# POSTECH-CVLab/RoDyGS

Hardware: AMD Instinct MI355X
Metric: train-step fps at 1M dynamic Gaussians / 1080p (fwd+bwd+Adam, one camera per GPU per step) (higher is better)
Workload: dtype f32; 1 GPU; 1000000 dynamic Gaussians + deformation MLP, 1920x1080, SH3, 100-frame synthetic video (BASELINE configs[2]); points=1000000, width=1920, height=1080, scene=uniform, frames=100, deferred_overflow_check=True, frame_order=orbit positions, bit-reversed, one_device=False, graph_replay=False, densify_stats=True, deterministic_backward=True, render_normal=True, parallelism=single GPU (frame-dp1), losses=photometric, sh_adam_in_backward=True, binning=bucket

## Files before the change

rodygs_amd/csrc/rdg_api.hip:

```cpp
#include "rdg_common.h"
#include <dlfcn.h>
#include <math.h>
#include <stdarg.h>
#include <stdio.h>
#include <string.h>
#include <stdlib.h>
#include <mutex>

static thread_local char g_err[512] = "";

int rdg_set_error(const char* fmt, ...) {
    va_list ap;
    va_start(ap, fmt);
    vsnprintf(g_err, sizeof(g_err), fmt, ap);
    va_end(ap);
    return -1;
}
int rdg_check_hip(hipError_t e, const char* what) {
    if (e == hipSuccess) return 0;
    return rdg_set_error("%s: %s", what, hipGetErrorString(e));
}

#define RDG_MAX_PENDING 4096
struct RdgPending { hipEvent_t a, b; int stage; };
// ... 57 lines not shown
    if (stage < 0 || stage >= RDG_STAGE_COUNT || !g_open[stage]) return;
    hipEvent_t e;
    if (hipEventCreate(&e) != hipSuccess) { (void)hipEventDestroy(g_open[stage]); g_open[stage] = nullptr; return; }
    (void)hipEventRecord(e, s);
    std::lock_guard<std::mutex> lk(g_timing_mu);
    if (g_npending >= RDG_MAX_PENDING) rdg_timing_drain();
    g_pending[g_npending].a = g_open[stage];
    g_pending[g_npending].b = e;
    g_pending[g_npending].stage = stage;
    g_npending++;
    g_open[stage] = nullptr;
}

void rdg_set_pose_aux(hipStream_t s);
int rdg_pose_fork_event_ready();

static int rdg_make_dev(const RdgRasterSettings* s, RdgDev* d) {
    if (!s) return rdg_set_error("settings pointer is NULL");
    if (s->P < 0 || s->image_height <= 0 || s->image_width <= 0) return rdg_set_error("bad sizes");
    if (s->sh_degree < 0 || s->sh_degree > 3) return rdg_set_error("sh_degree must be 0..3");
    d->P = s->P; d->M = s->M; d->deg = s->sh_degree; d->H = s->image_height; d->W = s->image_width;
    d->gx = (d->W + RDG_TILE - 1) / RDG_TILE; d->gy = (d->H + RDG_TILE - 1) / RDG_TILE;
    d->tanx = s->tanfovx; d->tany = s->tanfovy;
    d->fx = (float)((double)d->W / (2.0 * (double)s->tanfovx));
    d->fy = (float)((double)d->H / (2.0 * (double)s->tanfovy));
    d->smod = s->scale_modifier;
    d->prefiltered = s->prefiltered; d->cov_grad = s->enable_cov_grad; d->sh_grad = s->enable_sh_grad;
    d->render_normal = s->render_normal;
    d->cull = s->cull ? 1 : 0;
    d->bin_mode = s->bin_mode; d->nren_stats = s->num_rendered_stats; d->list_hints = s->list_hints;
// ... 69 lines not shown
    size_t cap = (size_t)(capacity > 0 ? capacity : 1);
    return rdg_align_up(cap * 8, 256) + rdg_align_up(cap * 4, 256) + rdg_sort_layout(capacity).total;
}

int rdg_preprocess_forward(const RdgRasterSettings* s_host, const float* means3D, const float* shs,
                           const float* colors_precomp, const float* opacities, const float* scales,
                           const float* rotations, const float* cov3D_precomp, const float* viewmatrix,
                           const float* projmatrix, void* geom_ws, int32_t* radii, int32_t* num_rendered_dev,
                           void* stream) {
    RdgDev d;
    if (rdg_make_dev(s_host, &d)) return -1;
    if (rdg_check_inputs(s_host, shs, colors_precomp, scales, rotations, cov3D_precomp)) return -1;
    hipStream_t st = (hipStream_t)stream;
    rdg_stage_begin(RDG_STAGE_PREPROCESS, st);
    int rc = rdg_launch_preprocess_fwd(d, means3D, shs, colors_precomp, opacities, scales, rotations, cov3D_precomp,
                                       viewmatrix, projmatrix, geom_ws, radii, num_rendered_dev, st);
    rdg_stage_end(RDG_STAGE_PREPROCESS, st);
    return rc;
}

int rdg_geom_from_records(const RdgRasterSettings* s_host, void* geom_ws, int32_t* radii, int32_t* num_rendered_dev,
                          void* stream) {
    RdgDev d;
    if (rdg_make_dev(s_host, &d)) return -1;
    if (!geom_ws || !radii || !num_rendered_dev) return rdg_set_error("rdg_geom_from_records: NULL argument");
    return rdg_launch_geom_from_records(d, geom_ws, radii, num_rendered_dev, (hipStream_t)stream);
}

int rdg_composite_forward(const RdgRasterSettings* s_host, const float* bg, const void* geom_ws, const int32_t* radii,
                          void* binning_ws, int64_t capacity, void* image_ws, int32_t* num_rendered_dev,
                          float* out_color, float* out_depth, float* out_normal, float* out_alpha, void* stream) {
// ... 8 lines not shown
    rdg_stage_end(RDG_STAGE_RENDER_FWD, st);
    return rc;
}

int rdg_rasterize_forward(const RdgRasterSettings* s_host, const float* bg, const float* means3D, const float* shs,
                          const float* colors_precomp, const float* opacities, const float* scales,
                          const float* rotations, const float* cov3D_precomp, const float* viewmatrix,
                          const float* projmatrix, void* geom_ws, void* binning_ws, int64_t capacity, void* image_ws,
                          float* out_color, float* out_depth, float* out_normal, float* out_alpha, int32_t* radii,
                          int32_t* num_rendered_dev, void* stream) {
    RdgDev d;
    if (rdg_make_dev(s_host, &d)) return -1;
    if (rdg_check_inputs(s_host, shs, colors_precomp, scales, rotations, cov3D_precomp)) return -1;
    hipStream_t st = (hipStream_t)stream;
    const RdgImageLayout I = rdg_image_layout(d.H, d.W);
    rdg_stage_begin(RDG_STAGE_PREPROCESS, st);
    int rc = rdg_launch_preprocess_fwd(d, means3D, shs, colors_precomp, opacities, scales, rotations, cov3D_precomp,
                                       viewmatrix, projmatrix, geom_ws, radii, num_rendered_dev, st,
                                       (uint32_t*)((char*)image_ws + I.tile_cnt), rdg_cnt_entries(d.gx, d.gy));
    rdg_stage_end(RDG_STAGE_PREPROCESS, st);
    if (rc) return rc;
    d.tile_cnt_zeroed = 1;
    rc = rdg_launch_bin(d, geom_ws, radii, binning_ws, capacity, image_ws, num_rendered_dev, nullptr, nullptr, st);
    if (rc) return rc;
    rdg_stage_begin(RDG_STAGE_RENDER_FWD, st);
    rc = rdg_launch_render_fwd(d, bg, geom_ws, binning_ws, capacity, image_ws, num_rendered_dev, out_color, out_depth,
                               out_normal, out_alpha, st);
    rdg_stage_end(RDG_STAGE_RENDER_FWD, st);
    return rc;
}

int rdg_composite_backward(const RdgRasterSettings* s_host, const float* bg, const void* geom_ws,
                           const void* binning_ws, int64_t capacity, const void* image_ws,
                           const float* grad_out_color, const float* grad_out_depth, const float* grad_out_alpha,
                           const float* grad_out_normal, void* grad_ws, void* stream) {
    RdgDev d;
    if (rdg_make_dev(s_host, &d)) return -1;
    hipStream_t st = (hipStream_t)stream;
// ... 354 lines not shown
```

rodygs_amd/csrc/rdg_common.h:

```cpp
#pragma once
#include <hip/hip_runtime.h>
#include <stdint.h>
#include <stddef.h>
#include "../../include/rodygs_hip.h"

#define RDG_TILE 16
#define RDG_TILE_PIX 256
#define RDG_WAVE 64

#define RDG_NEAR_CULL 0.2f
#define RDG_FOV_CLAMP 1.3f
#define RDG_DILATION 0.3f
#define RDG_ALPHA_CAP 0.99f
#define RDG_ALPHA_MIN (1.0f / 255.0f)
#define RDG_T_STOP 0.0001f
#define RDG_LAMBDA_FLOOR 0.1f

struct __attribute__((aligned(64))) RdgRec {
    float4 q0, q1, q2, q3;
};

#define RDG_GROW 16

static inline size_t rdg_align_up(size_t x, size_t a) { return (x + a - 1) / a * a; }
// ... 190 lines not shown
__device__ __forceinline__ RdgShAdam rdg_sh_adam_resolve(RdgShAdam ad) {
    if (ad.dev) {
        const float inv = ad.dev->inv_bias_correction1;
        const bool tab = ad.dev->lr_from_table != 0;
        ad.step_head = (tab ? ad.dev->sh_lr_head : ad.lr_head) * inv;
        ad.step_tail = (tab ? ad.dev->sh_lr_tail : ad.lr_tail) * inv;
        ad.bc2_sqrt = ad.dev->sqrt_bias_correction2;
    }
    return ad;
}
#endif

int rdg_launch_preprocess_fwd(const RdgDev& d, const float* means3D, const float* shs, const float* colors,
                              const float* opac, const float* scales, const float* rots, const float* cov3D,
                              const float* view, const float* proj, void* geom_ws, int32_t* radii,
                              int32_t* num_rendered, hipStream_t s, uint32_t* zero_buf = nullptr, size_t zero_words = 0);
int rdg_launch_densify_stats(long long n, long long row0, const float* dmeans2D, const int32_t* radii, float* accum,
                             float* denom, float* maxr, hipStream_t s);
int rdg_launch_geom_from_records(const RdgDev& d, void* geom_ws, int32_t* radii, int32_t* num_rendered,
                                 hipStream_t s);
int rdg_launch_bin(const RdgDev& d, const void* geom_ws, const int32_t* radii, void* bin_ws, int64_t capacity,
                   void* image_ws, int32_t* num_rendered, uint64_t* keys_unsorted_copy,
                   uint32_t* vals_unsorted_copy, hipStream_t s, bool export_sorted_keys = false);
int rdg_launch_sort(uint64_t* keys_a, uint64_t* keys_b, uint32_t* vals_a, uint32_t* vals_b, int64_t capacity,
                    const int32_t* n_dev, int end_bit, void* sort_tmp, int* result_in_b, hipStream_t s);
template <typename KeyT>
int rdg_launch_radix_sort(KeyT* keys_a, KeyT* keys_b, uint32_t* vals_a, uint32_t* vals_b, int64_t capacity,
                        const int32_t* n_dev, int begin_bit, int end_bit, void* tmp, int* result_in_b, hipStream_t s);
int rdg_launch_render_fwd(const RdgDev& d, const float* bg, const void* geom_ws, void* bin_ws,
                          int64_t capacity, void* image_ws, const int32_t* num_rendered, float* out_color,
                          float* out_depth, float* out_normal, float* out_alpha, hipStream_t s);
// ... 265 lines not shown
```

rodygs_amd/csrc/rdg_preprocess_fwd.hip:

```cpp
#include "rdg_common.h"

#define SH_C0 0.28209479177387814f
#define SH_C1 0.4886025119029199f
__device__ static const float SH_C2[5] = {1.0925484305920792f, -1.0925484305920792f, 0.31539156525252005f,
                                          -1.0925484305920792f, 0.5462742152960396f};
__device__ static const float SH_C3[7] = {-0.5900435899266435f, 2.890611442640554f, -0.4570457994644658f,
                                          0.3731763325901154f,  -0.4570457994644658f, 1.445305721320277f,
                                          -0.5900435899266435f};

__device__ __forceinline__ void rdg_rect(float px, float py, int radius, int gx, int gy, int& x0, int& y0,
                                         int& x1, int& y1) {
    float r = (float)radius;
    x0 = min(gx, max(0, (int)((px - r) / (float)RDG_TILE)));
    y0 = min(gy, max(0, (int)((py - r) / (float)RDG_TILE)));
    x1 = min(gx, max(0, (int)((((px + r) + (float)RDG_TILE) - 1.0f) / (float)RDG_TILE)));
    y1 = min(gy, max(0, (int)((((py + r) + (float)RDG_TILE) - 1.0f) / (float)RDG_TILE)));
}

__device__ __forceinline__ float rdg_ln_exact_ops(float x) {
    const uint32_t u = __float_as_uint(x);
    int e = (int)(u >> 23) - 127;
    float m = __uint_as_float((u & 0x007fffffu) | 0x3f800000u);
    if (m > 1.41421354f) { m = m * 0.5f; e += 1; }
    const float s = (m - 1.0f) / (m + 1.0f);
// ... 18 lines not shown
    const float cxx = (c_eff * cyy) / a;
    const float hx = sqrtf(r2 * cxx), hy = sqrtf(r2 * cyy);
    const float lox = fmaxf(ceilf(q0.x - hx), 0.0f), hix = fminf(floorf(q0.x + hx), (float)(gx * RDG_TILE - 1));
    const float loy = fmaxf(ceilf(q0.y - hy), 0.0f), hiy = fminf(floorf(q0.y + hy), (float)(gy * RDG_TILE - 1));
    if (hix < lox || hiy < loy) { x1 = x0; y1 = y0; return; }
    x0 = max(x0, (int)lox >> 4); x1 = min(x1, ((int)hix >> 4) + 1);
    y0 = max(y0, (int)loy >> 4); y1 = min(y1, ((int)hiy >> 4) + 1);
    if (x1 < x0) x1 = x0;
    if (y1 < y0) y1 = y0;
}
__device__ __forceinline__ uint4 rdg_pack_rectd(int x0, int y0, int x1, int y1, float depth, uint32_t tiles) {
    if (tiles == 0u) return make_uint4(0u, 0u, 0u, 0u);
    return make_uint4((uint32_t)x0 | ((uint32_t)y0 << 16), (uint32_t)x1 | ((uint32_t)y1 << 16), __float_as_uint(depth), tiles);
}

template <bool MULTI>
__global__ void __launch_bounds__(RDG_PRE_BLOCK)
rdg_preprocess_fwd_kernel(RdgDev d, const float* __restrict__ view_b, const float* __restrict__ proj,
                          const float* __restrict__ means3D_b, const float* __restrict__ shs,
                          const float* __restrict__ colors, const float* __restrict__ opac,
                          const float* __restrict__ scales, const float* __restrict__ rots_b,
                          const float* __restrict__ cov3Dp, RdgRec* __restrict__ rec_b,
                          uint32_t* __restrict__ tiles_touched_b, uint8_t* __restrict__ clampedm_b,
                          uint32_t* __restrict__ block_sums_b, int32_t* __restrict__ radii_b, int nviews_arg,
                          int vstride_arg, int blk0_arg, uint4* __restrict__ rectd_b) {
    const int nviews = MULTI ? nviews_arg : 1, vstride = MULTI ? vstride_arg : 0;
    const int bid = (MULTI ? blk0_arg : 0) + (int)blockIdx.x;
    const int i = bid * RDG_PRE_BLOCK + threadIdx.x;
    __shared__ float sSH[RDG_PRE_BLOCK / 64][64 * 49];
    const int sh_row = d.M * 3, sh_stride = sh_row | 1;
    const long long wave_first = (long long)bid * RDG_PRE_BLOCK + (threadIdx.x >> 6) * 64;
    if (shs && wave_first < d.P) {
        rdg_rows_to_lds(shs, wave_first, d.P, sh_row, sh_stride, sSH[threadIdx.x >> 6], threadIdx.x & 63);
        rdg_wave_lds_sync();
    }
    __shared__ uint32_t wsum[RDG_PRE_BLOCK / RDG_WAVE];
    for (int vw = 0; vw < nviews; ++vw) {
    const size_t vo = (size_t)vw * vstride;
    const float* __restrict__ view = view_b + 16 * vw;
    const float* __restrict__ means3D = means3D_b + vo * 3;
    const float* __restrict__ rots = rots_b ? rots_b + vo * 4 : nullptr;
    RdgRec* __restrict__ rec = rec_b + vo;
    uint32_t* __restrict__ tiles_touched = tiles_touched_b + vo;
    uint8_t* __restrict__ clampedm = clampedm_b + vo;
    int32_t* __restrict__ radii = radii_b + vo;
    uint32_t* __restrict__ block_sums = block_sums_b + vo / RDG_PRE_BLOCK;
    uint4* __restrict__ rectd = rectd_b + vo;
    float V[16], Pm[16];
#pragma unroll
    for (int k = 0; k < 16; ++k) { V[k] = view[k]; Pm[k] = proj[k]; }
    uint32_t my_tiles = 0;
    if (i < d.P) {
        int radius_out = 0;
        uint8_t cl = 0;
        uint4 rd = make_uint4(0u, 0u, 0u, 0u);
        RdgRec R;
        R.q0 = make_float4(0.f, 0.f, 0.f, 0.f);
        R.q1 = R.q0; R.q2 = R.q0; R.q3 = R.q0;
        const float x = means3D[3 * i + 0], y = means3D[3 * i + 1], z = means3D[3 * i + 2];
        const float vx = ((V[0] * x + V[4] * y) + V[8] * z) + V[12];
        const float vy = ((V[1] * x + V[5] * y) + V[9] * z) + V[13];
        const float vz = ((V[2] * x + V[6] * y) + V[10] * z) + V[14];
        bool valid = vz > RDG_NEAR_CULL;
        if (valid) {
            const float hx = ((Pm[0] * vx + Pm[4] * vy) + Pm[8] * vz) + Pm[12];
            const float hy = ((Pm[1] * vx + Pm[5] * vy) + Pm[9] * vz) + Pm[13];
            const float hw = ((Pm[3] * vx + Pm[7] * vy) + Pm[11] * vz) + Pm[15];
            const float pw = 1.0f / (hw + 1e-7f);
            const float ndc_x = hx * pw, ndc_y = hy * pw;

            float S00, S01, S02, S11, S12, S22;
            float nx = 0.f, ny = 0.f, nz = 0.f;
            if (cov3Dp) {
                S00 = cov3Dp[6 * i + 0]; S01 = cov3Dp[6 * i + 1]; S02 = cov3Dp[6 * i + 2];
                S11 = cov3Dp[6 * i + 3]; S12 = cov3Dp[6 * i + 4]; S22 = cov3Dp[6 * i + 5];
            } else {
                const float s0 = d.smod * scales[3 * i + 0], s1 = d.smod * scales[3 * i + 1],
                            s2 = d.smod * scales[3 * i + 2];
                const float4 q = reinterpret_cast<const float4*>(rots)[i];
                const float r = q.x, qx = q.y, qy = q.z, qz = q.w;
                const float R00 = 1.0f - 2.0f * (qy * qy + qz * qz), R01 = 2.0f * (qx * qy - r * qz),
                            R02 = 2.0f * (qx * qz + r * qy);
                const float R10 = 2.0f * (qx * qy + r * qz), R11 = 1.0f - 2.0f * (qx * qx + qz * qz),
                            R12 = 2.0f * (qy * qz - r * qx);
                const float R20 = 2.0f * (qx * qz - r * qy), R21 = 2.0f * (qy * qz + r * qx),
                            R22 = 1.0f - 2.0f * (qx * qx + qy * qy);
                const float L00 = R00 * s0, L01 = R01 * s1, L02 = R02 * s2;
                const float L10 = R10 * s0, L11 = R11 * s1, L12 = R12 * s2;
                const float L20 = R20 * s0, L21 = R21 * s1, L22 = R22 * s2;
                S00 = (L00 * L00 + L01 * L01) + L02 * L02;
                S01 = (L00 * L10 + L01 * L11) + L02 * L12;
                S02 = (L00 * L20 + L01 * L21) + L02 * L22;
                S11 = (L10 * L10 + L11 * L11) + L12 * L12;
                S12 = (L10 * L20 + L11 * L21) + L12 * L22;
                S22 = (L20 * L20 + L21 * L21) + L22 * L22;
                if (d.render_normal) {
                    const float sc0 = scales[3 * i + 0], sc1 = scales[3 * i + 1], sc2 = scales[3 * i + 2];
                    int k = 0; float sm = sc0;
                    if (sc1 < sm) { sm = sc1; k = 1; }
                    if (sc2 < sm) { sm = sc2; k = 2; }
                    const float n0 = k == 0 ? R00 : (k == 1 ? R01 : R02);
                    const float n1 = k == 0 ? R10 : (k == 1 ? R11 : R12);
                    const float n2 = k == 0 ? R20 : (k == 1 ? R21 : R22);
                    float nvx = (V[0] * n0 + V[4] * n1) + V[8] * n2;
                    float nvy = (V[1] * n0 + V[5] * n1) + V[9] * n2;
                    float nvz = (V[2] * n0 + V[6] * n1) + V[10] * n2;
                    const float dotv = (nvx * vx + nvy * vy) + nvz * vz;
                    const float sg = dotv > 0.f ? -1.0f : 1.0f;
                    nx = nvx * sg; ny = nvy * sg; nz = nvz * sg;
                }
            }
            const float limx = RDG_FOV_CLAMP * d.tanx, limy = RDG_FOV_CLAMP * d.tany;
// ... 12 lines not shown
            const float u12 = (T10 * S02 + T11 * S12) + T12 * S22;
            const float ca = ((u00 * T00 + u01 * T01) + u02 * T02) + RDG_DILATION;
            const float cb = (u00 * T10 + u01 * T11) + u02 * T12;
            const float cc = ((u10 * T10 + u11 * T11) + u12 * T12) + RDG_DILATION;
            const float det = ca * cc - cb * cb;
            valid = det != 0.0f;
            if (valid) {
                const float det_inv = 1.0f / det;
                const float mid = 0.5f * (ca + cc);
                const float disc = sqrtf(fmaxf(RDG_LAMBDA_FLOOR, mid * mid - det));
                const float lam = fmaxf(mid + disc, mid - disc);
                const int radius = (int)ceilf(3.0f * sqrtf(lam));
                const float px = ((ndc_x + 1.0f) * (float)d.W - 1.0f) * 0.5f;
                const float py = ((ndc_y + 1.0f) * (float)d.H - 1.0f) * 0.5f;
                const float4 rq0 = make_float4(px, py, cc * det_inv, -cb * det_inv);
                const float4 rq1 = make_float4(ca * det_inv, opac[i], vz, __int_as_float(radius));
                const float inv_cyy = 1.0f / cc;
                int x0, y0, x1, y1;
                rdg_rect(px, py, radius, d.gx, d.gy, x0, y0, x1, y1);
                const int area = (x1 - x0) * (y1 - y0);
                if (area > 0) {
                    if (d.cull) rdg_splat_rect(rq0, rq1, inv_cyy, d.gx, d.gy, 1, x0, y0, x1, y1);
                    my_tiles = (uint32_t)((x1 - x0) * (y1 - y0));
                    rd = rdg_pack_rectd(x0, y0, x1, y1, vz, my_tiles);
                    radius_out = radius;
                    float cr, cg, cbl;
                    if (colors) {
                        cr = colors[3 * i + 0]; cg = colors[3 * i + 1]; cbl = colors[3 * i + 2];
                    } else {
                        const float camx = -((V[0] * V[12] + V[1] * V[13]) + V[2] * V[14]);
                        const float camy = -((V[4] * V[12] + V[5] * V[13]) + V[6] * V[14]);
                        const float camz = -((V[8] * V[12] + V[9] * V[13]) + V[10] * V[14]);
                        float dx = x - camx, dy = y - camy, dz = z - camz;
                        const float ln = sqrtf((dx * dx + dy * dy) + dz * dz);
                        dx = dx / ln; dy = dy / ln; dz = dz / ln;
                        const float* sh = sSH[threadIdx.x >> 6] + (threadIdx.x & 63) * sh_stride;
                        float res[3];
#pragma unroll
                        for (int c = 0; c < 3; ++c) res[c] = SH_C0 * sh[c];
                        if (d.deg > 0) {
#pragma unroll
                            for (int c = 0; c < 3; ++c)
                                res[c] = res[c] - SH_C1 * dy * sh[3 + c] + SH_C1 * dz * sh[6 + c] -
                                         SH_C1 * dx * sh[9 + c];
                            if (d.deg > 1) {
                                const float xx = dx * dx, yy = dy * dy, zz = dz * dz;
                                const float xy = dx * dy, yz = dy * dz, xz = dx * dz;
#pragma unroll
                                for (int c = 0; c < 3; ++c)
                                    res[c] = res[c] + SH_C2[0] * xy * sh[12 + c] + SH_C2[1] * yz * sh[15 + c] +
                                             SH_C2[2] * (2.0f * zz - xx - yy) * sh[18 + c] +
                                             SH_C2[3] * xz * sh[21 + c] + SH_C2[4] * (xx - yy) * sh[24 + c];
                                if (d.deg > 2) {
#pragma unroll
                                    for (int c = 0; c < 3; ++c)
                                        res[c] = res[c] + SH_C3[0] * dy * (3.0f * xx - yy) * sh[27 + c] +
                                                 SH_C3[1] * xy * dz * sh[30 + c] +
                                                 SH_C3[2] * dy * (4.0f * zz - xx - yy) * sh[33 + c] +
                                                 SH_C3[3] * dz * (2.0f * zz - 3.0f * xx - 3.0f * yy) * sh[36 + c] +
                                                 SH_C3[4] * dx * (4.0f * zz - xx - yy) * sh[39 + c] +
                                                 SH_C3[5] * dz * (xx - yy) * sh[42 + c] +
                                                 SH_C3[6] * dx * (xx - 3.0f * yy) * sh[45 + c];
                                }
                            }
                        }
                        res[0] += 0.5f; res[1] += 0.5f; res[2] += 0.5f;
                        if (res[0] < 0.f) cl |= 1;
                        if (res[1] < 0.f) cl |= 2;
                        if (res[2] < 0.f) cl |= 4;
                        cr = fmaxf(res[0], 0.f); cg = fmaxf(res[1], 0.f); cbl = fmaxf(res[2], 0.f);
                    }
                    R.q0 = rq0;
                    R.q1 = rq1;
                    R.q2 = make_float4(cr, cg, cbl, inv_cyy);
                    R.q3 = make_float4(nx, ny, nz, 0.f);
                }
            }
        }
        rec[i] = R;
        tiles_touched[i] = my_tiles;
        rectd[i] = rd;
        clampedm[i] = cl;
        radii[i] = radius_out;
    }
    uint32_t inc = rdg_wave_scan_incl(my_tiles);
    const uint32_t lane = threadIdx.x & 63, w = threadIdx.x >> 6;
    if (lane == 63) wsum[w] = inc;
    __syncthreads();
    if (threadIdx.x == 0) block_sums[bid] = wsum[0] + wsum[1] + wsum[2] + wsum[3];
    if (nviews > 1) __syncthreads();
    }
}

__global__ void __launch_bounds__(1024) rdg_scan_block_sums_kernel(uint32_t* __restrict__ block_sums, int nblk,
                                                                   int32_t* __restrict__ num_rendered,
                                                                   uint32_t* __restrict__ zero_buf, int zero_words,
                                                                   int32_t* __restrict__ nren_max) {
    for (int i = threadIdx.x; i < zero_words; i += 1024) zero_buf[i] = 0u;
    __shared__ uint32_t wtot[16];
    __shared__ unsigned long long wtot64[16];
    const uint32_t lane = threadIdx.x & 63, w = threadIdx.x >> 6;
    const int per = (nblk + 1023) / 1024;
    const int t0 = min(nblk, (int)threadIdx.x * per), t1 = min(nblk, t0 + per);
    uint32_t mine = 0;
    unsigned long long mine64 = 0ull;
    for (int c0 = t0; c0 < t1; c0 += 8) {
// ... 68 lines not shown
    char* g = (char*)geom_ws;
    const int nblk = (d.P + RDG_PRE_BLOCK - 1) / RDG_PRE_BLOCK;
    uint32_t* block_sums = (uint32_t*)(g + L.block_sums);
    if (d.P > 0)
        hipLaunchKernelGGL(rdg_geom_from_records_kernel, dim3(nblk), dim3(RDG_PRE_BLOCK), 0, s, d.P, d.gx, d.gy, d.cull,
                           (const RdgRec*)(g + L.rec), (uint32_t*)(g + L.tiles_touched), block_sums, radii,
                           (uint4*)(g + L.rectd));
    hipLaunchKernelGGL(rdg_scan_block_sums_kernel, dim3(1), dim3(1024), 0, s, block_sums, d.P > 0 ? nblk : 0,
                       num_rendered, (uint32_t*)nullptr, 0, d.nren_max);
    return rdg_check_hip(hipGetLastError(), "geom_from_records launch");
}

int rdg_launch_preprocess_fwd(const RdgDev& d, const float* means3D, const float* shs, const float* colors,
                              const float* opac, const float* scales, const float* rots, const float* cov3D,
                              const float* view, const float* proj, void* geom_ws, int32_t* radii,
                              int32_t* num_rendered, hipStream_t s, uint32_t* zero_buf, size_t zero_words) {
    const RdgGeomLayout L = rdg_geom_layout(d.P);
    char* g = (char*)geom_ws;
    const int nblk = (d.P + RDG_PRE_BLOCK - 1) / RDG_PRE_BLOCK;
    uint32_t* block_sums = (uint32_t*)(g + L.block_sums);
    if (d.P > 0) {
        hipLaunchKernelGGL(rdg_preprocess_fwd_kernel<false>, dim3(nblk), dim3(RDG_PRE_BLOCK), 0, s, d, view, proj, means3D,
                           shs, colors, opac, scales, rots, cov3D, (RdgRec*)(g + L.rec),
                           (uint32_t*)(g + L.tiles_touched), (uint8_t*)(g + L.clamped), block_sums, radii, 1, 0, 0,
                           (uint4*)(g + L.rectd));
    }
    hipLaunchKernelGGL(rdg_scan_block_sums_kernel, dim3(1), dim3(1024), 0, s, block_sums, d.P > 0 ? nblk : 0,
                       num_rendered, zero_buf, (int)zero_words, d.nren_max);
    return rdg_check_hip(hipGetLastError(), "preprocess_fwd launch");
}

int rdg_launch_preprocess_fwd_views(const RdgDev& d_in, int32_t nviews, int32_t stride, int32_t row0,
                                    const float* means3D, const float* shs, const float* opac, const float* scales,
                                    const float* rots, const float* views, const float* proj, void* geom_ws,
                                    int32_t* radii, hipStream_t s) {
    const RdgGeomLayout L = rdg_geom_layout(nviews * stride);
// ... 13 lines not shown
```

rodygs_amd/rasterizer.py:

```python
from __future__ import annotations

import ctypes as C
import os
import threading
from typing import NamedTuple, Optional

import torch
import torch.nn as nn

from . import _lib

RENDER_NORMAL = True
PREZERO_GRAD_ROWS = os.environ.get("RDG_PREZERO_GRAD_ROWS", "1") != "0"
NREN_HOST_MIRROR = os.environ.get("RDG_NREN_MIRROR", "1") != "0"
BIN_RADIX_ABOVE = 32768
BIN_BUCKET_BELOW = 16384
BIN_RADIX_MEAN_LIST_ABOVE = 1000
BIN_BUCKET_MEAN_LIST_BELOW = 800
SPLIT_ABOVE = 4096
SPLIT_BELOW = 3072
_FORCE_RADIX = os.environ.get("RDG_BIN_MODE", "") == "radix"
_FORCE_BUCKET = os.environ.get("RDG_BIN_MODE", "") == "bucket"

DETERMINISTIC = os.environ.get("RDG_DETERMINISTIC", "0") == "1"
# ... 23 lines not shown
        self.capacity_hint = {}
        self.d_high = {}
        self.bin_hint = {}
        self.split_hint = {}
        self.pending = []
        self.pinned_free = []
        self.last_nren = None
        self.last_image = None
        self.graph_capture = False
        self.nren_max = None
        self.nren_max_key = None
        self.det_ws = None
        self.aux_stream = None
        self.pose_grad = None
        self.pose_fork_eager = None
        self.keep_alive = []
        self.lock = threading.RLock()

    def mode(self, name: str) -> bool:
        v = getattr(self, name)
        if v is not None:
            return bool(v)
        return bool({"deterministic": DETERMINISTIC, "force_radix": _FORCE_RADIX, "force_bucket": _FORCE_BUCKET,
                     "deferred_overflow_check": DEFERRED_OVERFLOW_CHECK, "render_normal": RENDER_NORMAL,
                     "cull": CULL}[name])

    def note_instances(self, key, n: int) -> None:
        self.d_high[key] = max(int(n), int(self.d_high.get(key, 0) * HINT_DECAY))

    def pinned_slot(self) -> torch.Tensor:
# ... 230 lines not shown
                cs.list_hints = 1 if det_mode else int(state.split_hint.get(key, 0))
                cap = max(int(state.capacity_hint.get(key, 0) * 1.25) + 4096, 4 * P + 4096)
                if capture and key not in state.capacity_hint:
                    raise RuntimeError("graph capture needs a warm-up forward of this (P, H, W) on the same RasterState first")
                deferred = state.mode("deferred_overflow_check") and key in state.capacity_hint and not capture
                if deferred:
                    state.poll_overflow(block=False)
                host = None
                if deferred:
                    host = state.pinned_slot()
                    host[0], host[1] = -1, -1
                    if NREN_HOST_MIRROR:
                        cs.num_rendered_host = host.data_ptr()
                if state.nren_max is not None and state.nren_max_key in (None, key):
                    cs.num_rendered_max = state.nren_max.data_ptr()
            while True:
                binning = torch.empty(L.rdg_binning_bytes(cap, n_tiles), **u8)
                rc = L.rdg_rasterize_forward(C.byref(cs), _lib.ptr(bg), _lib.ptr(m3), _lib.ptr(shs), _lib.ptr(col),
                                             _lib.ptr(op), _lib.ptr(sc), _lib.ptr(ro), _lib.ptr(cov), _lib.ptr(vm),
                                             _lib.ptr(pm), _lib.ptr(geom), _lib.ptr(binning), cap, _lib.ptr(image),
                                             _lib.ptr(color), _lib.ptr(depth), _lib.ptr(normal), _lib.ptr(alpha),
                                             _lib.ptr(radii), _lib.ptr(nren), stream)
                _lib.check(rc, "rdg_rasterize_forward")
                state.last_nren = (nren, key, cap)
                if capture:
                    n = -1
                    break
                if deferred:
                    if not NREN_HOST_MIRROR:
                        host.copy_(nren, non_blocking=True)
# ... 210 lines not shown
```

rodygs_amd/trainstep.py:

```python
from __future__ import annotations

import math
import os
from typing import Optional

import torch
import torch.nn.functional as F

from . import _lib
from .deform import (MLPBasisNetwork, dynamic_gaussians, dynamic_getter_supported, gaussian_deformation,
                     gaussian_deformation_packed)
from .dp import BucketedAllReduce, FlatParams, allreduce_sum_, frame_for
from .losses import fused_photometric_loss
from .model_ops import activate_gaussians, pose_view_matrix
from .rasterizer import GaussianRasterizationSettings, GaussianRasterizer, RasterState


def quaternion_to_matrix(q: torch.Tensor) -> torch.Tensor:
    r, i, j, k = q[0], q[1], q[2], q[3]
    two_s = 2.0 / (q * q).sum()
    return torch.stack([
        1 - two_s * (j * j + k * k), two_s * (i * j - k * r), two_s * (i * k + j * r),
        two_s * (i * j + k * r), 1 - two_s * (i * i + k * k), two_s * (j * k - i * r),
        two_s * (i * k - j * r), two_s * (j * k + i * r), 1 - two_s * (i * i + j * j)]).reshape(3, 3)
# ... 109 lines not shown
                h = ctypes.c_void_p()
                prio = int(os.environ.get("RDG_SIDE_STREAM_PRIORITY", str(least.value)))
                if hip.hipStreamCreateWithPriority(ctypes.byref(h), 1, prio) == 0 and h.value:
                    st = torch.cuda.ExternalStream(h.value, device=idx)
    except OSError:
        st = None
    if st is None:
        st = torch.cuda.Stream(device=idx)
    _LOW_PRIORITY_STREAMS[idx] = st
    return st


_FUSE_SH_ADAM = os.environ.get("RDG_FUSE_SH_ADAM", "1") != "0"
_EARLY_ROWS_ADAM = os.environ.get("RDG_EARLY_ROWS_ADAM", "1") != "0"
_EAGER_POSE_FORK = os.environ.get("RDG_EAGER_POSE_FORK", "1") != "0"
_PLAIN_FULL_FAST = os.environ.get("RDG_PLAIN_FULL_FAST", "1") != "0"

_MLP_SINK_ORDER = ("timenet.0.weight", "timenet.0.bias", "timenet.2.weight", "timenet.2.bias", "timenet.4.weight",
                   "timenet.4.bias", "head_w1", "head_b1", "head_w2", "head_b2")


def bind_module_to_flat(net: torch.nn.Module, lr: float, device, extra_spec=None) -> FlatParams:
    spec = {name: (tuple(p.shape), lr) for name, p in net.named_parameters()}
    spec.update(extra_spec or {})
    sp = FlatParams(spec, device)
    with torch.no_grad():
        for name, p in list(net.named_parameters()):
            sp[name].copy_(p)
            mod_name, _, leaf = name.rpartition(".")
            mod = net.get_submodule(mod_name) if mod_name else net
# ... 355 lines not shown
        main = torch.cuda.current_stream(self.device)
        if self._side_stream is None:
            self._side_stream = _low_priority_stream(self.device)
        side = self._side_stream
        side.wait_stream(main)
        with torch.cuda.stream(side):
            fused_adam_(self.fp, names=[k for k in self.fp.names if k != "features"])
        self._rows_stepped = True

    def train_step(self, step: int, rank: int = 0, world: int = 1, perm=None) -> torch.Tensor:
        perm = perm if perm is not None else list(self.gt.keys())
        frame = frame_for(step, rank, world, perm)
        after = None
        self._rows_adam_hook, self._rows_stepped = None, False
        self.raster_state.pose_fork_eager = None
        if self.full_losses and step % self.rigidity[1] != 0 and _PLAIN_FULL_FAST:
            fuse = world == 1 and _FUSE_SH_ADAM
            loss, after = self._full_loss_plain(frame, fuse)
        elif self.full_losses:
            loss = self._full_loss(step, frame)
        else:
            self.fuse_sh_adam = fuse = world == 1 and _FUSE_SH_ADAM
            eager = self._graph_inputs is None and not self.raster_state.graph_capture
            if fuse and _EARLY_ROWS_ADAM and eager:
                self._rows_adam_hook = self._step_rows_early
            if fuse and _EAGER_POSE_FORK and eager and self.pose_sinks is not None:
                if self._pose_fork is None:
                    self._pose_fork = (torch.cuda.Stream(device=self.device),
                                       torch.empty(4, 4, dtype=torch.float32, device=self.device))
                self.raster_state.pose_fork_eager = self._pose_fork
# ... 330 lines not shown
```

Before: 710.9 frames/s.

## Split SH colour evaluation from preprocess and overlap it with binning on aux stream

Splits the forward preprocess into a geometry-only kernel (no SH loads into LDS) and a separate colour kernel that evaluates SH for visible Gaussians. When an aux stream is available in eager mode, the colour kernel runs on that stream concurrently with binning, joined before render. The goal is to take the SH-to-RGB cost and its LDS footprint off the critical path. In exchange it adds an extra kernel launch, a second read of means, and event fork/join overhead, plus contention between streams.

```diff
diff --git a/rodygs_amd/csrc/rdg_api.hip b/rodygs_amd/csrc/rdg_api.hip
--- a/rodygs_amd/csrc/rdg_api.hip
+++ b/rodygs_amd/csrc/rdg_api.hip
@@ -95,6 +95,23 @@
 
 void rdg_set_pose_aux(hipStream_t s);
 int rdg_pose_fork_event_ready();
+
+static int rdg_fwd_split_colour() {
+    const char* e = getenv("RDG_FWD_SPLIT_COLOUR");
+    return e && e[0] == '0' ? 0 : (e && e[0] == '2' ? 2 : 1);
+}
+static thread_local hipEvent_t g_colour_fork_ev = nullptr, g_colour_join_ev = nullptr;
+static int rdg_colour_events_ready() {
+    if (!g_colour_fork_ev && hipEventCreateWithFlags(&g_colour_fork_ev, hipEventDisableTiming) != hipSuccess) {
+        g_colour_fork_ev = nullptr;
+        return rdg_set_error("colour fork: hipEventCreate failed");
+    }
+    if (!g_colour_join_ev && hipEventCreateWithFlags(&g_colour_join_ev, hipEventDisableTiming) != hipSuccess) {
+        g_colour_join_ev = nullptr;
+        return rdg_set_error("colour join: hipEventCreate failed");
+    }
+    return 0;
+}
 
 static int rdg_make_dev(const RdgRasterSettings* s, RdgDev* d) {
     if (!s) return rdg_set_error("settings pointer is NULL");
@@ -194,7 +211,8 @@
     hipStream_t st = (hipStream_t)stream;
     rdg_stage_begin(RDG_STAGE_PREPROCESS, st);
     int rc = rdg_launch_preprocess_fwd(d, means3D, shs, colors_precomp, opacities, scales, rotations, cov3D_precomp,
-                                       viewmatrix, projmatrix, geom_ws, radii, num_rendered_dev, st);
+                                       viewmatrix, projmatrix, geom_ws, radii, num_rendered_dev, st, nullptr, 0,
+                                       rdg_fwd_split_colour() == 2);
     rdg_stage_end(RDG_STAGE_PREPROCESS, st);
     return rc;
 }
@@ -233,14 +251,27 @@
     if (rdg_check_inputs(s_host, shs, colors_precomp, scales, rotations, cov3D_precomp)) return -1;
     hipStream_t st = (hipStream_t)stream;
     const RdgImageLayout I = rdg_image_layout(d.H, d.W);
+    const int split_mode = rdg_fwd_split_colour();
+    hipStream_t aux = nullptr;
+    if (split_mode && shs && !colors_precomp && d.P > 0 && s_host->aux_stream && (hipStream_t)s_host->aux_stream != st) {
+        hipStreamCaptureStatus cap_st = hipStreamCaptureStatusNone;
+        if (hipStreamIsCapturing(st, &cap_st) != hipSuccess) { (void)hipGetLastError(); cap_st = hipStreamCaptureStatusActive; }
+        if (cap_st == hipStreamCaptureStatusNone) {
+            if (rdg_colour_events_ready()) return -1;
+            aux = (hipStream_t)s_host->aux_stream;
+        }
+    }
+    const bool split = split_mode == 2 || aux != nullptr;
     rdg_stage_begin(RDG_STAGE_PREPROCESS, st);
     int rc = rdg_launch_preprocess_fwd(d, means3D, shs, colors_precomp, opacities, scales, rotations, cov3D_precomp,
                                        viewmatrix, projmatrix, geom_ws, radii, num_rendered_dev, st,
-                                       (uint32_t*)((char*)image_ws + I.tile_cnt), rdg_cnt_entries(d.gx, d.gy));
+                                       (uint32_t*)((char*)image_ws + I.tile_cnt), rdg_cnt_entries(d.gx, d.gy), split, aux,
+                                       g_colour_fork_ev, g_colour_join_ev);
     rdg_stage_end(RDG_STAGE_PREPROCESS, st);
-    if (rc) return rc;
+    if (rc) { if (aux) (void)hipStreamWaitEvent(st, g_colour_join_ev, 0); return rc; }
     d.tile_cnt_zeroed = 1;
     rc = rdg_launch_bin(d, geom_ws, radii, binning_ws, capacity, image_ws, num_rendered_dev, nullptr, nullptr, st);
+    if (aux && hipStreamWaitEvent(st, g_colour_join_ev, 0) != hipSuccess && !rc) rc = rdg_check_hip(hipGetLastError(), "colour join wait");
     if (rc) return rc;
     rdg_stage_begin(RDG_STAGE_RENDER_FWD, st);
     rc = rdg_launch_render_fwd(d, bg, geom_ws, binning_ws, capacity, image_ws, num_rendered_dev, out_color, out_depth,
diff --git a/rodygs_amd/csrc/rdg_common.h b/rodygs_amd/csrc/rdg_common.h
--- a/rodygs_amd/csrc/rdg_common.h
+++ b/rodygs_amd/csrc/rdg_common.h
@@ -228,7 +228,9 @@
 int rdg_launch_preprocess_fwd(const RdgDev& d, const float* means3D, const float* shs, const float* colors,
                               const float* opac, const float* scales, const float* rots, const float* cov3D,
                               const float* view, const float* proj, void* geom_ws, int32_t* radii,
-                              int32_t* num_rendered, hipStream_t s, uint32_t* zero_buf = nullptr, size_t zero_words = 0);
+                              int32_t* num_rendered, hipStream_t s, uint32_t* zero_buf = nullptr, size_t zero_words = 0,
+                              bool split_colour = false, hipStream_t colour_stream = nullptr, hipEvent_t fork_ev = nullptr,
+                              hipEvent_t join_ev = nullptr);
 int rdg_launch_densify_stats(long long n, long long row0, const float* dmeans2D, const int32_t* radii, float* accum,
                              float* denom, float* maxr, hipStream_t s);
 int rdg_launch_geom_from_records(const RdgDev& d, void* geom_ws, int32_t* radii, int32_t* num_rendered,
diff --git a/rodygs_amd/csrc/rdg_preprocess_fwd.hip b/rodygs_amd/csrc/rdg_preprocess_fwd.hip
--- a/rodygs_amd/csrc/rdg_preprocess_fwd.hip
+++ b/rodygs_amd/csrc/rdg_preprocess_fwd.hip
@@ -56,7 +56,53 @@
     return make_uint4((uint32_t)x0 | ((uint32_t)y0 << 16), (uint32_t)x1 | ((uint32_t)y1 << 16), __float_as_uint(depth), tiles);
 }
 
-template <bool MULTI>
+__device__ __forceinline__ uint8_t rdg_sh_to_rgb(int deg, const float (&V)[16], float x, float y, float z,
+                                                 const float* sh, float& cr, float& cg, float& cbl) {
+    const float camx = -((V[0] * V[12] + V[1] * V[13]) + V[2] * V[14]);
+    const float camy = -((V[4] * V[12] + V[5] * V[13]) + V[6] * V[14]);
+    const float camz = -((V[8] * V[12] + V[9] * V[13]) + V[10] * V[14]);
+    float dx = x - camx, dy = y - camy, dz = z - camz;
+    const float ln = sqrtf((dx * dx + dy * dy) + dz * dz);
+    dx = dx / ln; dy = dy / ln; dz = dz / ln;
+    float res[3];
+#pragma unroll
+    for (int c = 0; c < 3; ++c) res[c] = SH_C0 * sh[c];
+    if (deg > 0) {
+#pragma unroll
+        for (int c = 0; c < 3; ++c)
+            res[c] = res[c] - SH_C1 * dy * sh[3 + c] + SH_C1 * dz * sh[6 + c] -
+                     SH_C1 * dx * sh[9 + c];
+        if (deg > 1) {
+            const float xx = dx * dx, yy = dy * dy, zz = dz * dz;
+            const float xy = dx * dy, yz = dy * dz, xz = dx * dz;
+#pragma unroll
+            for (int c = 0; c < 3; ++c)
+                res[c] = res[c] + SH_C2[0] * xy * sh[12 + c] + SH_C2[1] * yz * sh[15 + c] +
+                         SH_C2[2] * (2.0f * zz - xx - yy) * sh[18 + c] +
+                         SH_C2[3] * xz * sh[21 + c] + SH_C2[4] * (xx - yy) * sh[24 + c];
+            if (deg > 2) {
+#pragma unroll
+                for (int c = 0; c < 3; ++c)
+                    res[c] = res[c] + SH_C3[0] * dy * (3.0f * xx - yy) * sh[27 + c] +
+                             SH_C3[1] * xy * dz * sh[30 + c] +
+                             SH_C3[2] * dy * (4.0f * zz - xx - yy) * sh[33 + c] +
+                             SH_C3[3] * dz * (2.0f * zz - 3.0f * xx - 3.0f * yy) * sh[36 + c] +
+                             SH_C3[4] * dx * (4.0f * zz - xx - yy) * sh[39 + c] +
+                             SH_C3[5] * dz * (xx - yy) * sh[42 + c] +
+                             SH_C3[6] * dx * (xx - 3.0f * yy) * sh[45 + c];
+            }
+        }
+    }
+    res[0] += 0.5f; res[1] += 0.5f; res[2] += 0.5f;
+    uint8_t cl = 0;
+    if (res[0] < 0.f) cl |= 1;
+    if (res[1] < 0.f) cl |= 2;
+    if (res[2] < 0.f) cl |= 4;
+    cr = fmaxf(res[0], 0.f); cg = fmaxf(res[1], 0.f); cbl = fmaxf(res[2], 0.f);
+    return cl;
+}
+
+template <bool MULTI, bool GEOM = false, bool COV = false>
 __global__ void __launch_bounds__(RDG_PRE_BLOCK)
 rdg_preprocess_fwd_kernel(RdgDev d, const float* __restrict__ view_b, const float* __restrict__ proj,
                           const float* __restrict__ means3D_b, const float* __restrict__ shs,
@@ -69,12 +115,15 @@
     const int nviews = MULTI ? nviews_arg : 1, vstride = MULTI ? vstride_arg : 0;
     const int bid = (MULTI ? blk0_arg : 0) + (int)blockIdx.x;
     const int i = bid * RDG_PRE_BLOCK + threadIdx.x;
-    __shared__ float sSH[RDG_PRE_BLOCK / 64][64 * 49];
+    static_assert(!(MULTI && GEOM), "the geometry kernel is single-camera");
+    __shared__ float sSH[GEOM ? 1 : RDG_PRE_BLOCK / 64][GEOM ? 1 : 64 * 49];
     const int sh_row = d.M * 3, sh_stride = sh_row | 1;
     const long long wave_first = (long long)bid * RDG_PRE_BLOCK + (threadIdx.x >> 6) * 64;
-    if (shs && wave_first < d.P) {
-        rdg_rows_to_lds(shs, wave_first, d.P, sh_row, sh_stride, sSH[threadIdx.x >> 6], threadIdx.x & 63);
-        rdg_wave_lds_sync();
+    if constexpr (!GEOM) {
+        if (shs && wave_first < d.P) {
+            rdg_rows_to_lds(shs, wave_first, d.P, sh_row, sh_stride, sSH[threadIdx.x >> 6], threadIdx.x & 63);
+            rdg_wave_lds_sync();
+        }
     }
     __shared__ uint32_t wsum[RDG_PRE_BLOCK / RDG_WAVE];
     for (int vw = 0; vw < nviews; ++vw) {
@@ -100,6 +149,25 @@
         R.q0 = make_float4(0.f, 0.f, 0.f, 0.f);
         R.q1 = R.q0; R.q2 = R.q0; R.q3 = R.q0;
         const float x = means3D[3 * i + 0], y = means3D[3 * i + 1], z = means3D[3 * i + 2];
+        float in_sc[3] = {0.f, 0.f, 0.f}, in_cov[6] = {0.f, 0.f, 0.f, 0.f, 0.f, 0.f}, in_op = 0.f;
+        float4 in_q = make_float4(0.f, 0.f, 0.f, 0.f);
+        const bool has_cov = GEOM ? COV : cov3Dp != nullptr;
+        if constexpr (GEOM) {
+            in_op = opac[i];
+            if constexpr (COV) {
+#pragma unroll
+                for (int k = 0; k < 6; ++k) in_cov[k] = cov3Dp[6 * i + k];
+            } else {
+                in_sc[0] = scales[3 * i + 0]; in_sc[1] = scales[3 * i + 1]; in_sc[2] = scales[3 * i + 2];
+                in_q = reinterpret_cast<const float4*>(rots)[i];
+            }
+            if constexpr (COV)
+                asm volatile("" ::"v"(in_op), "v"(in_cov[0]), "v"(in_cov[1]), "v"(in_cov[2]), "v"(in_cov[3]), "v"(in_cov[4]),
+                             "v"(in_cov[5]));
+            else
+                asm volatile("" ::"v"(in_op), "v"(in_sc[0]), "v"(in_sc[1]), "v"(in_sc[2]), "v"(in_q.x), "v"(in_q.y), "v"(in_q.z),
+                             "v"(in_q.w));
+        }
         const float vx = ((V[0] * x + V[4] * y) + V[8] * z) + V[12];
         const float vy = ((V[1] * x + V[5] * y) + V[9] * z) + V[13];
         const float vz = ((V[2] * x + V[6] * y) + V[10] * z) + V[14];
@@ -113,13 +181,20 @@
 
             float S00, S01, S02, S11, S12, S22;
             float nx = 0.f, ny = 0.f, nz = 0.f;
-            if (cov3Dp) {
-                S00 = cov3Dp[6 * i + 0]; S01 = cov3Dp[6 * i + 1]; S02 = cov3Dp[6 * i + 2];
-                S11 = cov3Dp[6 * i + 3]; S12 = cov3Dp[6 * i + 4]; S22 = cov3Dp[6 * i + 5];
+            if (has_cov) {
+                if constexpr (!GEOM) {
+#pragma unroll
+                    for (int k = 0; k < 6; ++k) in_cov[k] = cov3Dp[6 * i + k];
+                }
+                S00 = in_cov[0]; S01 = in_cov[1]; S02 = in_cov[2];
+                S11 = in_cov[3]; S12 = in_cov[4]; S22 = in_cov[5];
             } else {
-                const float s0 = d.smod * scales[3 * i + 0], s1 = d.smod * scales[3 * i + 1],
-                            s2 = d.smod * scales[3 * i + 2];
-                const float4 q = reinterpret_cast<const float4*>(rots)[i];
+                if constexpr (!GEOM) {
+                    in_sc[0] = scales[3 * i + 0]; in_sc[1] = scales[3 * i + 1]; in_sc[2] = scales[3 * i + 2];
+                    in_q = reinterpret_cast<const float4*>(rots)[i];
+                }
+                const float s0 = d.smod * in_sc[0], s1 = d.smod * in_sc[1], s2 = d.smod * in_sc[2];
+                const float4 q = in_q;
                 const float r = q.x, qx = q.y, qy = q.z, qz = q.w;
                 const float R00 = 1.0f - 2.0f * (qy * qy + qz * qz), R01 = 2.0f * (qx * qy - r * qz),
                             R02 = 2.0f * (qx * qz + r * qy);
@@ -137,7 +212,7 @@
                 S12 = (L10 * L20 + L11 * L21) + L12 * L22;
                 S22 = (L20 * L20 + L21 * L21) + L22 * L22;
                 if (d.render_normal) {
-                    const float sc0 = scales[3 * i + 0], sc1 = scales[3 * i + 1], sc2 = scales[3 * i + 2];
+                    const float sc0 = in_sc[0], sc1 = in_sc[1], sc2 = in_sc[2];
                     int k = 0; float sm = sc0;
                     if (sc1 < sm) { sm = sc1; k = 1; }
                     if (sc2 < sm) { sm = sc2; k = 2; }
@@ -180,7 +255,8 @@
                 const float px = ((ndc_x + 1.0f) * (float)d.W - 1.0f) * 0.5f;
                 const float py = ((ndc_y + 1.0f) * (float)d.H - 1.0f) * 0.5f;
                 const float4 rq0 = make_float4(px, py, cc * det_inv, -cb * det_inv);
-                const float4 rq1 = make_float4(ca * det_inv, opac[i], vz, __int_as_float(radius));
+                if constexpr (!GEOM) in_op = opac[i];
+                const float4 rq1 = make_float4(ca * det_inv, in_op, vz, __int_as_float(radius));
                 const float inv_cyy = 1.0f / cc;
                 int x0, y0, x1, y1;
                 rdg_rect(px, py, radius, d.gx, d.gy, x0, y0, x1, y1);
@@ -193,48 +269,11 @@
                     float cr, cg, cbl;
                     if (colors) {
                         cr = colors[3 * i + 0]; cg = colors[3 * i + 1]; cbl = colors[3 * i + 2];
+                    } else if constexpr (GEOM) {
+                        cr = cg = cbl = 0.f;
                     } else {
-                        const float camx = -((V[0] * V[12] + V[1] * V[13]) + V[2] * V[14]);
-                        const float camy = -((V[4] * V[12] + V[5] * V[13]) + V[6] * V[14]);
-                        const float camz = -((V[8] * V[12] + V[9] * V[13]) + V[10] * V[14]);
-                        float dx = x - camx, dy = y - camy, dz = z - camz;
-                        const float ln = sqrtf((dx * dx + dy * dy) + dz * dz);
-                        dx = dx / ln; dy = dy / ln; dz = dz / ln;
                         const float* sh = sSH[threadIdx.x >> 6] + (threadIdx.x & 63) * sh_stride;
-                        float res[3];
-#pragma unroll
-                        for (int c = 0; c < 3; ++c) res[c] = SH_C0 * sh[c];
-                        if (d.deg > 0) {
-#pragma unroll
-                            for (int c = 0; c < 3; ++c)
-                                res[c] = res[c] - SH_C1 * dy * sh[3 + c] + SH_C1 * dz * sh[6 + c] -
-                                         SH_C1 * dx * sh[9 + c];
-                            if (d.deg > 1) {
-                                const float xx = dx * dx, yy = dy * dy, zz = dz * dz;
-                                const float xy = dx * dy, yz = dy * dz, xz = dx * dz;
-#pragma unroll
-                                for (int c = 0; c < 3; ++c)
-                                    res[c] = res[c] + SH_C2[0] * xy * sh[12 + c] + SH_C2[1] * yz * sh[15 + c] +
-                                             SH_C2[2] * (2.0f * zz - xx - yy) * sh[18 + c] +
-                                             SH_C2[3] * xz * sh[21 + c] + SH_C2[4] * (xx - yy) * sh[24 + c];
-                                if (d.deg > 2) {
-#pragma unroll
-                                    for (int c = 0; c < 3; ++c)
-                                        res[c] = res[c] + SH_C3[0] * dy * (3.0f * xx - yy) * sh[27 + c] +
-                                                 SH_C3[1] * xy * dz * sh[30 + c] +
-                                                 SH_C3[2] * dy * (4.0f * zz - xx - yy) * sh[33 + c] +
-                                                 SH_C3[3] * dz * (2.0f * zz - 3.0f * xx - 3.0f * yy) * sh[36 + c] +
-                                                 SH_C3[4] * dx * (4.0f * zz - xx - yy) * sh[39 + c] +
-                                                 SH_C3[5] * dz * (xx - yy) * sh[42 + c] +
-                                                 SH_C3[6] * dx * (xx - 3.0f * yy) * sh[45 + c];
-                                }
-                            }
-                        }
-                        res[0] += 0.5f; res[1] += 0.5f; res[2] += 0.5f;
-                        if (res[0] < 0.f) cl |= 1;
-                        if (res[1] < 0.f) cl |= 2;
-                        if (res[2] < 0.f) cl |= 4;
-                        cr = fmaxf(res[0], 0.f); cg = fmaxf(res[1], 0.f); cbl = fmaxf(res[2], 0.f);
+                        cl = rdg_sh_to_rgb(d.deg, V, x, y, z, sh, cr, cg, cbl);
                     }
                     R.q0 = rq0;
                     R.q1 = rq1;
@@ -256,6 +295,42 @@
     if (threadIdx.x == 0) block_sums[bid] = wsum[0] + wsum[1] + wsum[2] + wsum[3];
     if (nviews > 1) __syncthreads();
     }
+}
+
+__global__ void __launch_bounds__(RDG_PRE_BLOCK)
+rdg_colour_fwd_kernel(int P, int M, int deg, const float* __restrict__ view, const float* __restrict__ means3D,
+                      const float* __restrict__ shs, const int32_t* __restrict__ radii, RdgRec* __restrict__ rec,
+                      uint8_t* __restrict__ clampedm) {
+    __shared__ float sSH[RDG_PRE_BLOCK / 64][64 * 49];
+    const int i = (int)blockIdx.x * RDG_PRE_BLOCK + (int)threadIdx.x;
+    const bool vis = i < P && radii[i] > 0;
+    if (__ballot(vis) == 0ull) return;
+    float x = 0.f, y = 0.f, z = 0.f;
+    if (vis) { x = means3D[3 * i + 0]; y = means3D[3 * i + 1]; z = means3D[3 * i + 2]; }
+    const int sh_row = M * 3, sh_stride = sh_row | 1;
+    const long long wave_first = (long long)blockIdx.x * RDG_PRE_BLOCK + (threadIdx.x >> 6) * 64;
+    rdg_rows_to_lds(shs, wave_first, P, sh_row, sh_stride, sSH[threadIdx.x >> 6], threadIdx.x & 63);
+    rdg_wave_lds_sync();
+    if (!vis) return;
+    float V[16];
+#pragma unroll
+    for (int k = 0; k < 16; ++k) V[k] = view[k];
+    float cr, cg, cbl;
+    const uint8_t cl = rdg_sh_to_rgb(deg, V, x, y, z, sSH[threadIdx.x >> 6] + (threadIdx.x & 63) * sh_stride, cr, cg, cbl);
+    float* q2 = reinterpret_cast<float*>(&rec[i].q2);
+    q2[0] = cr; q2[1] = cg; q2[2] = cbl;
+    clampedm[i] = cl;
+}
+
+int rdg_launch_colour_fwd(const RdgDev& d, const float* means3D, const float* shs, const float* view, void* geom_ws,
+                          const int32_t* radii, hipStream_t s) {
+    if (d.P <= 0) return 0;
+    const RdgGeomLayout L = rdg_geom_layout(d.P);
+    char* g = (char*)geom_ws;
+    const int nblk = (d.P + RDG_PRE_BLOCK - 1) / RDG_PRE_BLOCK;
+    hipLaunchKernelGGL(rdg_colour_fwd_kernel, dim3(nblk), dim3(RDG_PRE_BLOCK), 0, s, d.P, d.M, d.deg, view, means3D, shs,
+                       radii, (RdgRec*)(g + L.rec), (uint8_t*)(g + L.clamped));
+    return rdg_check_hip(hipGetLastError(), "colour_fwd launch");
 }
 
 __global__ void __launch_bounds__(1024) rdg_scan_block_sums_kernel(uint32_t* __restrict__ block_sums, int nblk,
@@ -354,12 +429,34 @@
 int rdg_launch_preprocess_fwd(const RdgDev& d, const float* means3D, const float* shs, const float* colors,
                               const float* opac, const float* scales, const float* rots, const float* cov3D,
                               const float* view, const float* proj, void* geom_ws, int32_t* radii,
-                              int32_t* num_rendered, hipStream_t s, uint32_t* zero_buf, size_t zero_words) {
+                              int32_t* num_rendered, hipStream_t s, uint32_t* zero_buf, size_t zero_words,
+                              bool split_colour, hipStream_t colour_stream, hipEvent_t fork_ev, hipEvent_t join_ev) {
     const RdgGeomLayout L = rdg_geom_layout(d.P);
     char* g = (char*)geom_ws;
     const int nblk = (d.P + RDG_PRE_BLOCK - 1) / RDG_PRE_BLOCK;
     uint32_t* block_sums = (uint32_t*)(g + L.block_sums);
-    if (d.P > 0) {
+    if (d.P > 0 && split_colour) {
+        if (cov3D)
+            hipLaunchKernelGGL((rdg_preprocess_fwd_kernel<false, true, true>), dim3(nblk), dim3(RDG_PRE_BLOCK), 0, s, d, view,
+                               proj, means3D, shs, colors, opac, scales, rots, cov3D, (RdgRec*)(g + L.rec),
+                               (uint32_t*)(g + L.tiles_touched), (uint8_t*)(g + L.clamped), block_sums, radii, 1, 0, 0,
+                               (uint4*)(g + L.rectd));
+        else
+            hipLaunchKernelGGL((rdg_preprocess_fwd_kernel<false, true, false>), dim3(nblk), dim3(RDG_PRE_BLOCK), 0, s, d, view,
+                               proj, means3D, shs, colors, opac, scales, rots, cov3D, (RdgRec*)(g + L.rec),
+                               (uint32_t*)(g + L.tiles_touched), (uint8_t*)(g + L.clamped), block_sums, radii, 1, 0, 0,
+                               (uint4*)(g + L.rectd));
+        if (shs && !colors) {
+            hipStream_t cs = s;
+            if (colour_stream && colour_stream != s) {
+                if (hipEventRecord(fork_ev, s) != hipSuccess || hipStreamWaitEvent(colour_stream, fork_ev, 0) != hipSuccess)
+                    return rdg_check_hip(hipGetLastError(), "colour fork");
+                cs = colour_stream;
+            }
+            if (rdg_launch_colour_fwd(d, means3D, shs, view, geom_ws, radii, cs)) return -1;
+            if (cs != s && hipEventRecord(join_ev, cs) != hipSuccess) return rdg_check_hip(hipGetLastError(), "colour join");
+        }
+    } else if (d.P > 0) {
         hipLaunchKernelGGL(rdg_preprocess_fwd_kernel<false>, dim3(nblk), dim3(RDG_PRE_BLOCK), 0, s, d, view, proj, means3D,
                            shs, colors, opac, scales, rots, cov3D, (RdgRec*)(g + L.rec),
                            (uint32_t*)(g + L.tiles_touched), (uint8_t*)(g + L.clamped), block_sums, radii, 1, 0, 0,
diff --git a/rodygs_amd/rasterizer.py b/rodygs_amd/rasterizer.py
--- a/rodygs_amd/rasterizer.py
+++ b/rodygs_amd/rasterizer.py
@@ -61,6 +61,7 @@
         self.aux_stream = None
         self.pose_grad = None
         self.pose_fork_eager = None
+        self.fwd_aux = None
         self.keep_alive = []
         self.lock = threading.RLock()
 
@@ -321,6 +322,8 @@
                         cs.num_rendered_host = host.data_ptr()
                 if state.nren_max is not None and state.nren_max_key in (None, key):
                     cs.num_rendered_max = state.nren_max.data_ptr()
+                if state.fwd_aux is not None and not capture and not det_mode:
+                    cs.aux_stream = state.fwd_aux.cuda_stream
             while True:
                 binning = torch.empty(L.rdg_binning_bytes(cap, n_tiles), **u8)
                 rc = L.rdg_rasterize_forward(C.byref(cs), _lib.ptr(bg), _lib.ptr(m3), _lib.ptr(shs), _lib.ptr(col),
diff --git a/rodygs_amd/trainstep.py b/rodygs_amd/trainstep.py
--- a/rodygs_amd/trainstep.py
+++ b/rodygs_amd/trainstep.py
@@ -147,6 +147,7 @@
 _FUSE_SH_ADAM = os.environ.get("RDG_FUSE_SH_ADAM", "1") != "0"
 _EARLY_ROWS_ADAM = os.environ.get("RDG_EARLY_ROWS_ADAM", "1") != "0"
 _EAGER_POSE_FORK = os.environ.get("RDG_EAGER_POSE_FORK", "1") != "0"
+_FWD_COLOUR_AUX = os.environ.get("RDG_FWD_COLOUR_AUX", "1") != "0"
 _PLAIN_FULL_FAST = os.environ.get("RDG_PLAIN_FULL_FAST", "1") != "0"
 
 _MLP_SINK_ORDER = ("timenet.0.weight", "timenet.0.bias", "timenet.2.weight", "timenet.2.bias", "timenet.4.weight",
@@ -532,6 +533,12 @@
         after = None
         self._rows_adam_hook, self._rows_stepped = None, False
         self.raster_state.pose_fork_eager = None
+        self.raster_state.fwd_aux = None
+        if _FWD_COLOUR_AUX and self._graph_inputs is None and not self.raster_state.graph_capture:
+            if self._pose_fork is not None:
+                self.raster_state.fwd_aux = self._pose_fork[0]
+            elif self._side_stream is not None:
+                self.raster_state.fwd_aux = self._side_stream
         if self.full_losses and step % self.rigidity[1] != 0 and _PLAIN_FULL_FAST:
             fuse = world == 1 and _FUSE_SH_ADAM
             loss, after = self._full_loss_plain(frame, fuse)
```

Result: no change. 716.5 frames/s, median of 6 (+0.8%).
